# themayflyman/yet-another-raytracer

Hardware: AMD Instinct MI355X
Metric: Msamples/sec (WxHxspp/sec), cornell-box 800x800x256spp depth 50 (higher is better)
Workload: dtype f64; 1 GPU; cornell-box 800x800x256spp depth 50 (BASELINE configs[1]); width=800, height=800, spp=256, max_depth=50, parallelism=pixel-blocks x1, launch=one process, one GPU, streams=2, prep_frames=0, full=False, seed=1497453140, build_id=b5b5abf84520346f09e41dc92cfc8f159110369d6109f06c5935a081cd03fc2a

## Files before the change

yet-another-raytracer_amd/csrc/kernels.hip:

```cpp
#include <hip/hip_runtime.h>
#include <math.h>
#include <type_traits>

#include "kernels.h"

namespace yart_dev {

__constant__ double c_cie[471][3] = {
#include "cie_xyz.inc"
};
constexpr double kMinLambda = 360.0, kMaxLambda = 720.0, kBinWidth = 10.0;
constexpr double kCieYIntegral = 106.856895;
constexpr double kMaxLum = 20.0;
constexpr double kPi = 3.141592653589793;
constexpr double kEps = 2.220446049250313e-16;
constexpr double kF64Max = 1.7976931348623157e308;

struct V3 { double x, y, z; };
__device__ __forceinline__ V3 mk(double x, double y, double z) { return V3{x, y, z}; }
__device__ __forceinline__ V3 add(V3 a, V3 b) { return mk(a.x + b.x, a.y + b.y, a.z + b.z); }
__device__ __forceinline__ V3 sub(V3 a, V3 b) { return mk(a.x - b.x, a.y - b.y, a.z - b.z); }
__device__ __forceinline__ V3 muls(V3 a, double s) { return mk(a.x * s, a.y * s, a.z * s); }
__device__ __forceinline__ V3 smul(double s, V3 a) { return mk(s * a.x, s * a.y, s * a.z); }
__device__ __forceinline__ V3 neg(V3 a) { return mk(-a.x, -a.y, -a.z); }
// ... 1532 lines not shown
      cx(0, 1); cx(2, 3); cx(0, 2); cx(1, 3); cx(1, 2);
      if (key[0] < INFINITY) {
        if (key[3] < INFINITY) stk[(cursor++) * 64] = hc[3];
        if (key[2] < INFINITY) stk[(cursor++) * 64] = hc[2];
        if (key[1] < INFINITY) stk[(cursor++) * 64] = hc[1];
        hnd = hc[0];
      } else {
        if (cursor == 0) break;
        cursor--;
        hnd = stk[cursor * 64];
      }
    }
  }
  id.obj = who >> 3; id.sub = who & 7u;
  id.t = closest;
  return found;
}

template <bool HAS_MESH, bool BVH, bool STATS, bool EXT, int SLOTS = kCoopSlots, bool OVF = false, bool PARK = false>
__device__ __forceinline__ bool world_hit(const DevScene& S, bool want, const Ray& r, double tmin, double tmax, Hit& rec,
                                          int32_t& which, uint32_t* stk, uint8_t* coop, Stats& st, const QueryCtx& q,
                                          uint32_t* ovf = nullptr, bool resume = false, bool* parked = nullptr) {
  HitId id;
  if constexpr (BVH) {
    if (!world_closest_bvh<STATS>(S, r, tmin, tmax, id, stk, st)) return false;
  } else {
    if (!world_closest<HAS_MESH, STATS, EXT, SLOTS, OVF, PARK>(S, want, r, tmin, tmax, id, stk, coop, st, q, ovf, resume, parked) ||
        !want || (PARK && *parked))
      return false;
  }
  hit_record<HAS_MESH, EXT>(S, r, id, rec);
  which = (int32_t)id.obj;
  return true;
}


struct Onb { V3 v, w; };
template <class M>
__device__ __forceinline__ Onb onb_from_w(V3 n, M& m) {
  Onb b;
  b.w = m.unit(n);
  const V3 a = fabs(b.w.x) > 0.9 ? mk(0.0, 1.0, 0.0) : mk(1.0, 0.0, 0.0);
  b.v = m.unit(cross(b.w, a));
  return b;
}
__device__ __forceinline__ V3 local(const Onb& b, V3 a) {
  const V3 u = cross(b.w, b.v);
  return add(add(smul(a.x, u), smul(a.y, b.v)), smul(a.z, b.w));
}
template <class M>
__device__ __forceinline__ V3 random_cosine_direction(Rng& g, M& m) {
  const double r1 = gen_f64(g), r2 = gen_f64(g);
  const double z = m.sqrt(1.0 - r2);
  double s, c;
  sincos_det(2.0 * kPi * r1, s, c);
  const double sr2 = m.sqrt(r2);
  return mk(c * sr2, s * sr2, z);
}
template <bool CDIV, class M>
__device__ __forceinline__ double over_pi(double x, M& m) {
  if (!CDIV || !YART_CONST_DIV) return x / kPi;
  double d = kPi, r = kRcpPi;
  asm volatile("" : "+s"(d), "+s"(r));
  return m.quo(x, PosDen{d, r});
}
template <bool CDIV, class M>
__device__ __forceinline__ double cosine_value(const Onb& b, V3 ud, M& m) {
  const double cosine = dot(ud, b.w);
  return cosine <= 0.0 ? 0.0 : over_pi<CDIV>(cosine, m);
}

template <bool LEN, class M>
__device__ __forceinline__ double light_pdf_at(const DevObject& o, V3 origin, V3 dir, double ldir, bool hit, double t, M& m) {
  if (!hit) return 0.0;
  if (o.kind == YART_PRIM_XZ_RECT) {
    Hit h;
    rect_rec(1, Ray{origin, dir, 0.0, 0.0}, t, h);
    const double area = (o.p[1] - o.p[0]) * (o.p[3] - o.p[2]);
    const double distance_squared = h.t * h.t * len2(dir);
    const double cosine = fabs(dot(dir, h.n)) / (LEN ? m.len(dir) : ldir);
    return distance_squared / (cosine * area);
  }
  const double radius = o.p[3];
  const double cos_theta_max = m.sqrt(1.0 - radius * radius / len2(sub(ld3(o.p), origin)));
  const double solid_angle = 2.0 * kPi * (1.0 - cos_theta_max);
  return 1.0 / solid_angle;
}
template <bool STATS, bool LEN, class M>
__device__ __forceinline__ double light_pdf(const DevObject& o, V3 origin, V3 dir, double ldir, double wl, Stats& st, M& m) {
  if (o.n_xf != 0) return 0.0;
  Ray r{origin, dir, 0.0, wl};
  double t = 0.0;
  bool hit;
  if (o.kind == YART_PRIM_XZ_RECT) {
    if (STATS) st.v[ST_LIGHT]++;
    hit = rect_t<1, 0, 2>(o.p, r, 0.001, INFINITY, t);
  } else if (o.kind == YART_PRIM_SPHERE) {
    if (STATS) st.v[ST_LIGHT]++;
    hit = sphere_t(o.p, r, 0.001, INFINITY, t, m);
  } else {
    return 0.0;
  }
  return light_pdf_at<LEN>(o, origin, dir, ldir, hit, t, m);
}
template <class M>
__device__ __forceinline__ V3 light_random(const DevObject& o, V3 origin, Rng& g, M& m) {
  if (o.n_xf == 0 && o.kind == YART_PRIM_XZ_RECT) {
    const double x = gen_range(g, o.p[0], o.p[1]);
    const double z = gen_range(g, o.p[2], o.p[3]);
    return sub(mk(x, o.p[4], z), origin);
  }
  if (o.n_xf == 0 && o.kind == YART_PRIM_SPHERE) {
    const V3 direction = sub(ld3(o.p), origin);
    const double d2 = len2(direction);
    const Onb uvw = onb_from_w(direction, m);
    const double r1 = gen_f64(g), r2 = gen_f64(g);
    const double radius = o.p[3];
    const double z = 1.0 + r2 * (m.sqrt(1.0 - radius * radius / d2) - 1.0);
    double s, c;
    sincos_det(2.0 * kPi * r1, s, c);
    const double sz = m.sqrt(1.0 - z * z);
    const V3 rs = mk(c * sz, s * sz, z);
    return local(uvw, rs);
  }
  return mk(1.0, 0.0, 0.0);
}

__device__ __forceinline__ int32_t sat_i32(double f) {
  if (f != f) return 0;
  if (f >= 2147483647.0) return INT32_MAX;
  if (f <= -2147483648.0) return INT32_MIN;
  return (int32_t)f;
}
__device__ __noinline__ double perlin_noise(const yart_perlin* P, uint32_t type, V3 p) {
  if (type == YART_NOISE_SQUARE) {
    const int32_t i = sat_i32(4.0 * p.x) & 255, j = sat_i32(4.0 * p.y) & 255, k = sat_i32(4.0 * p.z) & 255;
    return P->ranfloat[P->perm_x[i] ^ P->perm_y[j] ^ P->perm_z[k]];
  }
  double u = p.x - floor(p.x), v = p.y - floor(p.y), w = p.z - floor(p.z);
  const uint32_t i = (uint32_t)sat_i32(floor(p.x)), j = (uint32_t)sat_i32(floor(p.y)), k = (uint32_t)sat_i32(floor(p.z));
  double accum = 0.0;
  if (type == YART_NOISE_TRILINEAR) {
    u = u * u * (3.0 - 2.0 * u);
    v = v * v * (3.0 - 2.0 * v);
    w = w * w * (3.0 - 2.0 * w);
    for (uint32_t di = 0; di < 2; ++di)
      for (uint32_t dj = 0; dj < 2; ++dj)
        for (uint32_t dk = 0; dk < 2; ++dk) {
          const double c = P->ranfloat[P->perm_x[(i + di) & 255u] ^ P->perm_y[(j + dj) & 255u] ^ P->perm_z[(k + dk) & 255u]];
          accum += ((double)di * u + (double)(1u - di) * (1.0 - u)) * ((double)dj * v + (double)(1u - dj) * (1.0 - v)) *
                   ((double)dk * w + (double)(1u - dk) * (1.0 - w)) * c;
        }
    return accum;
  }
  const double uu = u * u * (3.0 - 2.0 * u), vv = v * v * (3.0 - 2.0 * v), ww = w * w * (3.0 - 2.0 * w);
  for (uint32_t di = 0; di < 2; ++di)
    for (uint32_t dj = 0; dj < 2; ++dj)
      for (uint32_t dk = 0; dk < 2; ++dk) {
        const double* c = P->ranvec[P->perm_x[(i + di) & 255u] ^ P->perm_y[(j + dj) & 255u] ^ P->perm_z[(k + dk) & 255u]];
        const V3 weight_v = mk(u - (double)di, v - (double)dj, w - (double)dk);
        accum += ((double)di * uu + (1.0 - (double)di) * (1.0 - uu)) * ((double)dj * vv + (1.0 - (double)dj) * (1.0 - vv)) *
                 ((double)dk * ww + (1.0 - (double)dk) * (1.0 - ww)) * dot(weight_v, ld3(c));
      }
  return accum;
}
__device__ __forceinline__ double perlin_turb(const yart_perlin* P, uint32_t type, V3 p, int depth) {
  double accum = 0.0, weight = 1.0;
  V3 temp_p = p;
  for (int d = 0; d < depth; ++d) {
    accum += weight * perlin_noise(P, type, temp_p);
    weight *= 0.5;
    temp_p = muls(temp_p, 2.0);
  }
  return fabs(accum);
}

__constant__ double c_smits[7][36] = {
#include "smits.inc"
};
__device__ __forceinline__ double rgb_reflect(double red, double green, double blue, int i) {
  enum { W, Cy, Ma, Ye, Re, Gr, Bl };
  double s = 0.0;
  if (red <= green && red <= blue) {
    s = red * c_smits[W][i] + s;
    if (green <= blue) { s = (green - red) * c_smits[Cy][i] + s; s = (blue - green) * c_smits[Bl][i] + s; }
    else { s = (blue - red) * c_smits[Cy][i] + s; s = (green - blue) * c_smits[Gr][i] + s; }
  } else if (green <= red && green <= blue) {
    s = green * c_smits[W][i] + s;
    if (red <= blue) { s = (red - green) * c_smits[Ma][i] + s; s = (blue - red) * c_smits[Bl][i] + s; }
    else { s = (blue - green) * c_smits[Ma][i] + s; s = (red - blue) * c_smits[Re][i] + s; }
  } else {
    s = blue * c_smits[W][i] + s;
    if (red <= green) { s = (red - blue) * c_smits[Ye][i] + s; s = (green - red) * c_smits[Gr][i] + s; }
    else { s = (green - blue) * c_smits[Ye][i] + s; s = (red - green) * c_smits[Re][i] + s; }
  }
  return s;
}
__device__ __forceinline__ double clampd(double x, double lo, double hi) { return x < lo ? lo : (x > hi ? hi : x); }
__device__ __forceinline__ uint32_t sat_u32(double f) {
  if (!(f > 0.0)) return 0u;
  if (f >= 4294967295.0) return 0xFFFFFFFFu;
  return (uint32_t)f;
}

template <bool EXT>
__device__ __forceinline__ double texture_value(const DevScene& S, uint32_t ti, int bin, V3 p, double hu = 0.0,
                                                double hv = 0.0) {
  const DevTexture& t = S.textures[ti];
  if (EXT && t.kind == YART_TEX_IMAGE) {
    if (!t.pixels || t.width == 0 || t.height == 0) return 1.0;
    const double uu = clampd(hu, 0.0, 1.0), vv = 1.0 - clampd(hv, 0.0, 1.0);
    uint32_t i = sat_u32(uu * (double)t.width), j = sat_u32(vv * (double)t.height);
    if (i >= t.width) i = t.width - 1;
    if (j >= t.height) j = t.height - 1;
    const double color_scale = 1.0 / 255.0;
    const uint8_t* px = t.pixels + (size_t)j * t.width * 3 + (size_t)i * 3;
    return rgb_reflect(color_scale * (double)px[0], color_scale * (double)px[1], color_scale * (double)px[2], bin);
  }
  if (EXT && t.kind == YART_TEX_NOISE) {
    const double white = t.spec[bin];
    if (t.noise_type == YART_NOISE_NET) return white * perlin_turb(t.perlin, t.noise_type, muls(p, t.scale), 7);
    if (t.noise_type == YART_NOISE_MARBLE)
      return white * 0.5 * (1.0 + sin_det(t.scale * p.z + 10.0 * perlin_turb(t.perlin, t.noise_type, p, 7)));
    return white * 0.5 * (1.0 + perlin_noise(t.perlin, t.noise_type, muls(p, t.scale)));
  }
  if (t.kind == YART_TEX_CHECKER) {
    const double sines = sin_det(10.0 * p.x) * sin_det(10.0 * p.y) * sin_det(10.0 * p.z);
    return sines < 0.0 ? t.spec[bin] : t.spec_even[bin];
  }
  return t.spec[bin];
}
__device__ __forceinline__ V3 reflect(V3 v, V3 n) { return sub(v, smul(2.0 * dot(v, n), n)); }

constexpr size_t kKernargCam = (sizeof(DevScene) + alignof(RenderArgs) - 1) / alignof(RenderArgs) * alignof(RenderArgs) +
                               offsetof(RenderArgs, cam);
typedef const __attribute__((address_space(4))) yart_camera* kcam_ptr;
__device__ __forceinline__ kcam_ptr kernarg_camera() {
  const __attribute__((address_space(4))) char* p =
      (const __attribute__((address_space(4))) char*)__builtin_amdgcn_kernarg_segment_ptr();
  asm volatile("" : "+s"(p));
  return (kcam_ptr)(p + kKernargCam);
}
__device__ __forceinline__ V3 ld3(const __attribute__((address_space(4))) double* p) { return mk(p[0], p[1], p[2]); }
#ifndef YART_KA_OPAQUE
#define YART_KA_OPAQUE 1
#endif
typedef const __attribute__((address_space(4))) RenderArgs* kargs_ptr;
template <bool OPAQUE>
__device__ __forceinline__ kargs_ptr kernarg_args() {
  const __attribute__((address_space(4))) char* p =
      (const __attribute__((address_space(4))) char*)__builtin_amdgcn_kernarg_segment_ptr();
  if (OPAQUE) asm volatile("" : "+s"(p));
  return (kargs_ptr)(p + (kKernargCam - offsetof(RenderArgs, cam)));
}

template <class Cam>
__device__ __forceinline__ Ray camera_ray(const Cam& c, double s, double t, double wl, Rng& g,
                                          bool draw_time) {
  const V3 org = ld3(c.origin);
  const V3 d0 = sub(add(add(ld3(c.lower_left_corner), smul(s, ld3(c.horizontal))), smul(t, ld3(c.vertical))), org);
  Ray r;
  r.wl = wl;
  if (c.lens_radius == 0.0 && !draw_time && org.x != 0.0 && org.y != 0.0 && org.z != 0.0 && d0.x != 0.0 &&
      d0.y != 0.0 && d0.z != 0.0) {
    r.o = org;
    r.d = d0;
    r.time = c.time0;
    return r;
  }
  V3 p;
  for (int guard = 0; guard < 1024; ++guard) {
    const double x = gen_range(g, -1.0, 1.0);
    const double y = gen_range(g, -1.0, 1.0);
    p = mk(x, y, 0.0);
    if (!(len2(p) >= 1.0)) break;
  }
  const V3 rd = smul(c.lens_radius, p);
  const V3 offset = add(muls(ld3(c.u), rd.x), muls(ld3(c.v), rd.y));
  r.o = add(org, offset);
  r.d = sub(d0, offset);
  r.time = draw_time ? gen_range(g, c.time0, c.time1) : c.time0;
  return r;
}

__device__ __forceinline__ bool covered(uint32_t x, uint32_t w) {
  asm volatile("" : "+s"(w));
  const uint32_t cw = w / 8;
#pragma unroll
  for (uint32_t col = 0; col < 8; ++col) {
    const uint32_t x0 = (uint32_t)(((uint64_t)w * col) / 8);
    if (x >= x0 && x < x0 + cw) return true;
  }
  return false;
}

__device__ __forceinline__ uint32_t xcd_remap(uint32_t b, uint32_t n) {
  const uint32_t q = n / 8, r = n % 8, xcd = b % 8, k = b / 8;
  return (xcd < r ? xcd * (q + 1) : r * (q + 1) + (xcd - r) * q) + k;
}

constexpr int kWavesPerEu = 4;
constexpr int kMeshWavesPerEu = 4;

template <bool EXT, bool STATS, bool SHARE, class MP>
__device__ __forceinline__ void scatter_at(const DevScene& S, MP& mp, Rng& g, const V3& hp, const V3& hn, uint32_t hmat,
                                           double hu, double hv, int wbin, const Ray& ray, double T, uint32_t depth,
                                           Stats& st, double& T_, V3& o_, V3& d_, uint32_t& depth_, double& R_,
                                           bool& term_) {
  T_ = T; o_ = hp; d_ = ray.d; depth_ = depth; R_ = 0.0; term_ = false;
  const DevMaterial& m = S.materials[hmat];
  const uint32_t kind = m.kind;
  if (kind == YART_MAT_LAMBERTIAN) {
    auto att = [&]() { return texture_value<EXT>(S, m.texture, wbin, hp, hu, hv); };
    const Onb uvw = onb_from_w(hn, mp);
    V3 dir, udir;
    double ldir;
    double pdf_val;
    if (S.n_lights == 0) {
      (void)gen_range(g, 0.0, 1.0);
      dir = local(uvw, random_cosine_direction(g, mp));
      udir = mp.unit_len(dir, ldir);
      pdf_val = 0.5 * cosine_value<SHARE && !EXT>(uvw, udir, mp) + 0.5 * cosine_value<SHARE && !EXT>(uvw, udir, mp);
    } else {
      if (gen_range(g, 0.0, 1.0) < 0.5) {
        if (S.n_lights <= 2) {
          dir = light_random(uniform_at(S.lights, 0u), hp, g, mp);
        } else {
          const uint32_t k = (uint32_t)gen_index(g, S.n_lights - 1);
          dir = light_random(S.lights[k], hp, g, mp);
        }
      } else {
        dir = local(uvw, random_cosine_direction(g, mp));
      }
      const double weight = 1.0 / (double)S.n_lights;
      double sum = -0.0;
      if (SHARE) udir = mp.unit_len(dir, ldir);
      else ldir = 0.0;
      for (uint32_t i = 0; i < S.n_lights; ++i)
        sum = sum + weight * light_pdf<STATS, !SHARE>(uniform_at(S.lights, i), hp, dir, ldir, ray.wl, st, mp);
      if (!SHARE) udir = mp.unit(dir);
      pdf_val = 0.5 * sum + 0.5 * cosine_value<SHARE && !EXT>(uvw, udir, mp);
    }
    if (!isfinite(pdf_val) || pdf_val <= 0.0) {
      R_ = T * 0.0;
      term_ = true;
    } else {
      const double cosine = dot(hn, SHARE ? udir : mp.unit(dir));
      const double spdf = cosine < 0.0 ? 0.0 : over_pi<SHARE && !EXT>(cosine, mp);
      T_ = ((T * att()) * spdf) / pdf_val;
      o_ = hp;
      d_ = dir;
      depth_ = depth - 1;
    }
  } else if (EXT && kind == YART_MAT_ISOTROPIC) {
    const double att = texture_value<EXT>(S, m.texture, wbin, hp, hu, hv);
    V3 p;
    for (int guard = 0; guard < 1024; ++guard) {
      const double px = gen_range(g, -1.0, 1.0), py = gen_range(g, -1.0, 1.0), pz = gen_range(g, -1.0, 1.0);
      p = mk(px, py, pz);
      if (!(len2(p) >= 1.0)) break;
    }
    T_ = T * att;
    o_ = hp;
    d_ = p;
    depth_ = depth - 1;
  } else if (kind == YART_MAT_METAL) {
    const V3 reflected = reflect(mp.unit(ray.d), hn);
    V3 p;
    for (int guard = 0; guard < 1024; ++guard) {
      const double px = gen_range(g, -1.0, 1.0), py = gen_range(g, -1.0, 1.0), pz = gen_range(g, -1.0, 1.0);
      p = mk(px, py, pz);
      if (!(len2(p) >= 1.0)) break;
    }
    const double att = texture_value<EXT>(S, m.texture, wbin, hp, hu, hv);
    T_ = T * att;
    o_ = hp;
    d_ = add(reflected, smul(m.fuzz, p));
    depth_ = depth - 1;
  } else {
    const double wl2 = ray.wl * ray.wl;
    const double n2 = 1.0 + m.b[0] * wl2 / (wl2 - m.c[0]) + m.b[1] * wl2 / (wl2 - m.c[1]) + m.b[2] * wl2 / (wl2 - m.c[2]);
    const double n = mp.sqrt(n2);
    const PosDen ld = mp.den(mp.len(ray.d));
    V3 outward;
    double ni_over_nt, cosine;
    if (dot(ray.d, hn) > 0.0) {
      outward = neg(hn); ni_over_nt = n; cosine = mp.quo(n * dot(ray.d, hn), ld);
    } else {
      outward = hn; ni_over_nt = 1.0 / n; cosine = mp.quo(-dot(ray.d, hn), ld);
    }
    const V3 uv = mk(mp.quo(ray.d.x, ld), mp.quo(ray.d.y, ld), mp.quo(ray.d.z, ld));
    const double dt = dot(uv, outward);
    const double disc = 1.0 - ni_over_nt * ni_over_nt * (1.0 - dt * dt);
    V3 out;
    if (disc > 0.0) {
      const V3 refracted = sub(muls(sub(uv, muls(outward, dt)), ni_over_nt), muls(outward, mp.sqrt(disc)));
      double r0 = (1.0 - n) / (1.0 + n);
      r0 = r0 * r0;
      const double sch = r0 + (1.0 - r0) * powi5(1.0 - cosine);
      out = gen_f64(g) < sch ? reflect(ray.d, hn) : refracted;
    } else {
      out = reflect(ray.d, hn);
    }
    T_ = T * 1.0;
    o_ = hp;
    d_ = out;
    depth_ = depth - 1;
  }
}

template <bool HAS_MESH, bool BVH, bool STATS, bool DYN, bool EXT, bool DEEP = false>
__global__ __launch_bounds__(256, HAS_MESH ? kMeshWavesPerEu : kWavesPerEu) void k_render(DevScene S, RenderArgs A_) {
#if YART_KA_OPAQUE
#define A (*kernarg_args<!BVH>())
#else
#define A A_
#endif
  __shared__ uint32_t s_stack[HAS_MESH ? 4 * kWaveLdsWords : BVH ? 4 * kStackSlots * 64 : 1];
  constexpr bool JOBL = DYN && !HAS_MESH, JOBL3 = DYN && HAS_MESH;
  constexpr bool PARK = HAS_MESH && DYN && !EXT && !DEEP;
  __shared__ uint32_t s_job[JOBL ? 4 * 6 * 64 : JOBL3 ? 4 * 3 * 64 : 1];
  const uint32_t lane = threadIdx.x & 63u, wave = __builtin_amdgcn_readfirstlane(threadIdx.x >> 6);
  uint32_t work = DYN ? 0u : xcd_remap(blockIdx.x, gridDim.x) * 4 + wave;
  if (!DYN && work >= A.n_blocks * A.n_chunks) return;
  uint32_t local_blk = work % A.n_blocks, chunk_id = work / A.n_blocks;
  uint32_t b = A.shard_index + local_blk * A.shard_count;
  uint32_t bx0 = (b % A.blocks_x) * 8, by0 = (b / A.blocks_x) * 8;
  uint32_t slot = lane;
  uint32_t x = bx0 + (slot & 7u), y = by0 + (slot >> 3);
  const uint32_t W = A.width, H = A.height;
  const bool active = x < W && y < H && covered(x, W) && covered(y, H);
  uint32_t* const jl = &s_job[JOBL ? wave * 6 * 64 + lane : JOBL3 ? wave * 3 * 64 + lane : 0];
  constexpr bool JL = JOBL || JOBL3;
  uint32_t* stk = &s_stack[HAS_MESH ? (wave * kWaveLdsWords + lane) : BVH ? (wave * kStackSlots * 64 + lane) : 0];
  uint8_t* coop = reinterpret_cast<uint8_t*>(&s_stack[HAS_MESH ? wave * kWaveLdsWords : 0]);
  uint32_t* const ovf = (DEEP || PARK) ? A.stack_ovf + (size_t)(blockIdx.x * 4u + wave) * kOvfWords : nullptr;
  if (PARK) {
    if (lane < 16u) reinterpret_cast<uint32_t*>(coop + coop_bytes<kCoopSlots>() + 64)[lane] = 0u;
    __builtin_amdgcn_fence(__ATOMIC_SEQ_CST, "wavefront");
  }
  Stats st;
  if (STATS) for (int i = 0; i < kNumStats; ++i) st.v[i] = 0;

  uint32_t pixel = y * W + x;
  double acc0 = 0.0, acc1 = 0.0, acc2 = 0.0;
  const uint32_t s_end = A.s_begin + A.s_count;
  uint32_t s_lo = A.s_begin + chunk_id * A.chunk;
  const uint32_t s_stop = s_lo + A.chunk < s_end ? s_lo + A.chunk : s_end;
  uint32_t smp = s_lo;
  uint32_t lane_blk = local_blk;
  uint32_t n_jobs = 0, next_job = 0;
  uint64_t cov = 0;
  bool drained = false;
  bool need = true;
  bool parked = false;
  bool alive = DYN ? true : (active && smp < s_stop);
  Rng g;
  Ray ray;
  double T = 1.0;
  uint32_t depth = 0;
  bool fresh = !DYN && alive;
  V3 hp = mk(0.0, 0.0, 0.0), hn = hp;
  uint32_t hmat = 0;
  double hu = 0.0, hv = 0.0;
  int wbin = 0;
  g.k0 = (uint32_t)A.seed; g.k1 = (uint32_t)(A.seed >> 32);

  for (;;) {
    if (DYN) {
      uint64_t m = drained ? 0ull : __ballot(need);
      while (m) {
        if (next_job >= n_jobs) {
          const uint32_t first = (uint32_t)__builtin_ctzll(__ballot(true));
          uint32_t v = 0;
          if (lane == first) {
            if (HAS_MESH) {
              v = 0xFFFFFFFFu;
              const uint32_t x0 = blockIdx.x & 7u;
              for (uint32_t k = 0; k < 8u; ++k) {
                const uint32_t x = (x0 + k) & 7u;
                const uint32_t lo = (uint32_t)(((uint64_t)A.n_units * x) >> 3);
                const uint32_t hi = (uint32_t)(((uint64_t)A.n_units * (x + 1u)) >> 3);
                if (hi <= lo) continue;
                const uint32_t t = atomicAdd(A.queue + 1 + x, 1u);
                if (t < hi - lo) { v = lo + t; break; }
              }
              if (A.progress) {
                const uint32_t c = v < A.n_units ? atomicAdd(A.queue, 1u) + 1u : A.n_units;
                __hip_atomic_store(A.progress, A.progress_base + (c < A.n_units ? c : A.n_units), __ATOMIC_RELAXED,
                                   __HIP_MEMORY_SCOPE_SYSTEM);
              }
            } else {
              v = atomicAdd(A.queue, 1u);
              if (A.progress)
                __hip_atomic_store(A.progress, A.progress_base + (v < A.n_units ? v + 1u : A.n_units), __ATOMIC_RELAXED,
                                   __HIP_MEMORY_SCOPE_SYSTEM);
            }
          }
          const uint32_t u = (uint32_t)__builtin_amdgcn_readlane((int)v, (int)first);
          if (u >= A.n_units) { drained = true; break; }
          local_blk = u / A.n_chunks; chunk_id = u % A.n_chunks;
          b = A.shard_index + local_blk * A.shard_count;
          bx0 = (b % A.blocks_x) * 8; by0 = (b / A.blocks_x) * 8;
          s_lo = A.s_begin + chunk_id * A.chunk;
          const uint32_t stop = s_lo + A.chunk < s_end ? s_lo + A.chunk : s_end;
          n_jobs = (stop > s_lo ? stop - s_lo : 0) * 64;
          next_job = 0;
          {
            const uint32_t cx = bx0 + (lane & 7u), cy = by0 + (lane >> 3);
            cov = __ballot(cx < W && cy < H && covered(cx, W) && covered(cy, H));
          }
          continue;
        }
        const uint32_t rank = __builtin_amdgcn_mbcnt_hi((uint32_t)(m >> 32), __builtin_amdgcn_mbcnt_lo((uint32_t)m, 0u));
        const uint32_t avail = n_jobs - next_job;
        if (need && rank < avail) {
          const uint32_t job = next_job + rank;
          slot = job & 63u;
          smp = s_lo + (job >> 6);
          x = bx0 + (slot & 7u);
          y = by0 + (slot >> 3);
          pixel = y * W + x;
          lane_blk = local_blk;
          if (JOBL) { jl[0] = pixel; jl[64] = smp; jl[128] = lane_blk; jl[192] = slot; jl[256] = x; jl[320] = y; }
          if (JOBL3) { jl[0] = pixel; jl[64] = smp; jl[128] = lane_blk; }
          if ((cov >> slot) & 1ull) { fresh = true; need = false; }
        }
        const uint32_t given = (uint32_t)__popcll(m);
        next_job += given < avail ? given : avail;
        m = __ballot(need);
      }
    }
    const bool run = DYN ? !need : alive;
    if (__ballot(run) == 0) break;
    bool term = false, want = PARK && parked;
    if (STATS) {
      const uint64_t cam = __ballot(run && fresh), sca = __ballot(run && !fresh);
      if (lane == 0) {
        st.v[ST_ITERS]++;
        st.v[ST_CAMERA_LANES] += (uint32_t)__popcll(cam);
        st.v[ST_SCATTER_LANES] += (uint32_t)__popcll(sca);
        st.v[ST_CAMERA_ITERS] += cam ? 1u : 0u;
        st.v[ST_SCATTER_ITERS] += sca ? 1u : 0u;
      }
    }
    if (run && !(PARK && parked)) {
      rng_phase<!HAS_MESH && !BVH>(g, JL ? jl[0] : pixel, JL ? jl[64] : smp, fresh ? 0u : A.max_depth - depth + 1u);
      if (fresh) {
        uint32_t jx = x, jy = y;
        if (JOBL) { jx = jl[256]; jy = jl[320]; }
        if (JOBL3) { const uint32_t p = jl[0]; jy = p / W; jx = p - jy * W; }
        uint32_t wm1 = W - 1, hm1 = H - 1;
        asm volatile("" : "+s"(wm1), "+s"(hm1));
        const double tx = (double)jx + gen_f64(g);
        const double u = tx / (double)wm1;
        const double ty = (double)jy + gen_f64(g);
        const double v = 1.0 - ty / (double)hm1;
        const double wl = gen_range(g, kMinLambda, kMaxLambda);
        ray = camera_ray(*kernarg_camera(), u, v, wl, g, EXT && S.has_time);
        wbin = spectrum_bin<!HAS_MESH && !EXT>(wl);
        T = 1.0;
        depth = A.max_depth;
        fresh = false;
      } else {
        auto scatter = [&](auto& mp, double& T_, V3& o_, V3& d_, uint32_t& depth_, double& R_, bool& term_) {
          scatter_at<EXT, STATS, !HAS_MESH>(S, mp, g, hp, hn, hmat, hu, hv, wbin, ray, T, depth, st, T_, o_, d_, depth_, R_, term_);
        };
        double nT, nR;
        V3 no, nd;
        uint32_t ndepth;
        bool nterm;
        typename MathPolicy<HAS_MESH, BVH, EXT>::type fm;
        scatter(fm, nT, no, nd, ndepth, nR, nterm);
        if (flagged(fm)) {
          rng_phase<!HAS_MESH && !BVH>(g, JL ? jl[0] : pixel, JL ? jl[64] : smp, A.max_depth - depth + 1u);
          Ieee im;
          scatter(im, nT, no, nd, ndepth, nR, nterm);
        }
        T = nterm ? nR : nT; ray.o = no; ray.d = nd; depth = ndepth; term = nterm;
      }
      if (!term) {
        if (depth == 0) {
          T = T * 1.0;
          term = true;
        } else {
          want = true;
        }
      }
    }
    {
      Hit h;
      int32_t which;
      bool hit = false;
      bool scat = false;
      const QueryCtx q{g.k0, g.k1, JL ? jl[64] : smp, JL ? jl[0] : pixel, A.max_depth - depth + 1u};
      if (HAS_MESH) {
        bool now = false;
        hit = world_hit<HAS_MESH, BVH, STATS, EXT, kCoopSlots, DEEP, PARK>(S, want, ray, 0.001, INFINITY, h, which, stk, coop, st, q,
                                                                          ovf, parked, &now);
        if (PARK) {
          parked = now;
          want = want && !now;
        }
      } else if (want) {
        hit = world_hit<HAS_MESH, BVH, STATS, EXT>(S, true, ray, 0.001, INFINITY, h, which, stk, coop, st, q);
      }
      if (want && !term) {
        if (STATS) st.v[ST_SEGMENTS]++;
        if (!hit) {
          T = T * S.background[wbin];
          term = true;
        } else {
          const DevMaterial& m = S.materials[h.mat];
          const uint32_t kind = m.kind;
          if (kind == YART_MAT_LAMBERTIAN || kind == YART_MAT_METAL || kind == YART_MAT_DIELECTRIC ||
              (EXT && kind == YART_MAT_ISOTROPIC)) {
            scat = true;
          } else {
            double emitted = 0.0;
            if (kind == YART_MAT_DIFFUSE_LIGHT && h.ff) emitted = texture_value<EXT>(S, m.texture, wbin, h.p, h.u, h.v);
            T = T * emitted;
            term = true;
          }
        }
      }
      hp = scat ? h.p : mk(0.0, 0.0, 0.0);
      hn = scat ? h.n : mk(0.0, 0.0, 0.0);
      hmat = scat ? h.mat : 0u;
      if (EXT) { hu = scat ? h.u : 0.0; hv = scat ? h.v : 0.0; }
    }
    if (run && term) {
      const double R = T;
      double cx, cy, cz;
      cie_xyz(ray.wl, cx, cy, cz);
      double sx = cx * R, sy = cy * R, sz = cz * R;
      if (!isfinite(sx) || !isfinite(sy) || !isfinite(sz)) {
        sx = sy = sz = 0.0;
      } else if (!(sy <= 0.0 || sy <= kMaxLum)) {
        const double k = kMaxLum / sy;
        sx = sx * k; sy = sy * k; sz = sz * k;
      }
      if (STATS) st.v[ST_SAMPLES]++;
      if (DYN) {
        const uint32_t jb = JL ? jl[128] : lane_blk, js = JL ? jl[64] : smp;
        uint32_t jsl = JOBL ? jl[192] : slot;
        if (JOBL3) {
          const uint32_t p = jl[0], py = p / W, px = p - py * W;
          jsl = (py & 7u) * 8u + (px & 7u);
        }
        double* q = A.scratch + 3 * (((size_t)jb * A.s_count + (js - A.s_begin)) * 64 + jsl);
        q[0] = sx; q[1] = sy; q[2] = sz;
        need = true;
      } else {
        acc0 = acc0 + sx; acc1 = acc1 + sy; acc2 = acc2 + sz;
        smp++;
        if (smp < s_stop) fresh = true;
        else alive = false;
      }
    }
  }
  if (!DYN && active) {
    double* o = A.out + 3 * (A.packed ? (size_t)local_blk * 64 + lane : (size_t)pixel);
    o[0] = acc0; o[1] = acc1; o[2] = acc2;
  }
  if (!DYN && A.progress && lane == 0) {
    const uint32_t done = atomicAdd(A.progress_count, 1u) + 1u;
    __hip_atomic_store(A.progress, A.progress_base + done, __ATOMIC_RELAXED, __HIP_MEMORY_SCOPE_SYSTEM);
  }
  if (STATS) {
    for (int i = 0; i < kNumStats; ++i)
      if (st.v[i]) atomicAdd(&A.stats[i], st.v[i]);
  }
}

#undef A

__device__ __forceinline__ void wf_job(const RenderArgs& A, uint32_t job, uint32_t& pixel, uint32_t& smp, uint32_t& x,
                                       uint32_t& y) {
  const uint32_t slot = job & 63u, rest = job >> 6;
  const uint32_t blk = rest / A.s_count, s = rest - blk * A.s_count;
  const uint32_t b = A.shard_index + blk * A.shard_count;
  x = (b % A.blocks_x) * 8u + (slot & 7u);
  y = (b / A.blocks_x) * 8u + (slot >> 3);
  pixel = y * A.width + x;
  smp = A.s_begin + s;
}
__device__ __forceinline__ void wf_store_sample(const RenderArgs& A, uint32_t job, double wl, double R) {
  double cx, cy, cz;
  cie_xyz(wl, cx, cy, cz);
  double sx = cx * R, sy = cy * R, sz = cz * R;
  if (!isfinite(sx) || !isfinite(sy) || !isfinite(sz)) {
    sx = sy = sz = 0.0;
  } else if (!(sy <= 0.0 || sy <= kMaxLum)) {
    const double k = kMaxLum / sy;
    sx = sx * k; sy = sy * k; sz = sz * k;
  }
  double* q = A.scratch + 3 * (size_t)job;
  q[0] = sx; q[1] = sy; q[2] = sz;
}

__global__ __launch_bounds__(256) void k_wf_shade(DevScene S, RenderArgs A, WfArgs F) {
  __shared__ uint32_t s_need[4], s_take[3];
  const uint32_t i = blockIdx.x * 256u + threadIdx.x;
  const uint32_t lane = threadIdx.x & 63u, wave = __builtin_amdgcn_readfirstlane(threadIdx.x >> 6);
  const uint32_t P = F.pool;
  const uint32_t W = A.width, H = A.height;
  const WfSlots& Q = F.q;
  Stats st;
  Rng g;
  g.k0 = (uint32_t)A.seed; g.k1 = (uint32_t)(A.seed >> 32);
  Ray ray;
  ray.time = 0.0;
  ray.wl = 0.0;
  ray.o = mk(0.0, 0.0, 0.0); ray.d = ray.o;
  double T = 0.0;
  uint32_t job = Q.job[i], depth = 0;
  bool has = false;
  if (job != kWfNoJob) {
    depth = Q.depth[i]; T = Q.T[i]; ray.wl = Q.wl[i];
    ray.o = mk(Q.o[i], Q.o[P + i], Q.o[2 * (size_t)P + i]);
    ray.d = mk(Q.d[i], Q.d[P + i], Q.d[2 * (size_t)P + i]);
    const int wbin = spectrum_bin<false>(ray.wl);
    const uint32_t obj = Q.hobj[i];
    double R = 0.0;
    bool term = false;
    if (obj == kWfMiss) {
      R = T * S.background[wbin];
      term = true;
    } else {
      HitId id;
      id.t = Q.ht[i]; id.u = Q.hu[i]; id.v = Q.hv[i]; id.obj = obj; id.sub = Q.hsub[i];
      Hit h;
      hit_record<true, false>(S, ray, id, h);
      const DevMaterial& m = S.materials[h.mat];
      const uint32_t kind = m.kind;
      if (kind == YART_MAT_LAMBERTIAN || kind == YART_MAT_METAL || kind == YART_MAT_DIELECTRIC) {
        uint32_t pixel, smp, x, y;
        wf_job(A, job, pixel, smp, x, y);
        rng_phase<false>(g, pixel, smp, A.max_depth - depth + 1u);
        double nT, nR;
        V3 no, nd;
        uint32_t ndepth;
        bool nterm;
        Ieee im;
        scatter_at<false, false, false>(S, im, g, h.p, h.n, h.mat, 0.0, 0.0, wbin, ray, T, depth, st, nT, no, nd, ndepth, nR, nterm);
        if (nterm) {
          R = nR;
          term = true;
        } else if (ndepth == 0) {
          R = nT * 1.0;
          term = true;
        } else {
          T = nT; ray.o = no; ray.d = nd; depth = ndepth;
          has = true;
        }
      } else {
        double emitted = 0.0;
        if (kind == YART_MAT_DIFFUSE_LIGHT && h.ff) emitted = texture_value<false>(S, m.texture, wbin, h.p);
        R = T * emitted;
        term = true;
      }
    }
    if (term) wf_store_sample(A, job, ray.wl, R);
  }
  bool need = !has;
  uint32_t next = 0, end = 0;
  if (threadIdx.x == 0) { next = Q.range[2 * blockIdx.x]; end = Q.range[2 * blockIdx.x + 1]; }
  for (;;) {
    if (!__syncthreads_or(need)) break;
    const uint64_t m = __ballot(need);
    if (lane == 0) s_need[wave] = (uint32_t)__popcll(m);
    __syncthreads();
    const uint32_t total = s_need[0] + s_need[1] + s_need[2] + s_need[3];
    uint32_t before = 0;
    for (uint32_t w = 0; w < wave; ++w) before += s_need[w];
    if (threadIdx.x == 0) {
      uint32_t base = kWfNoJob;
      if (end - next < total && *(volatile uint32_t*)F.jobs < F.total_jobs) {
        base = atomicAdd(F.jobs, kWfChunk);
        if (base >= F.total_jobs) base = kWfNoJob;
      }
      s_take[0] = next; s_take[1] = base;
      const uint32_t rem = end - next;
      if (base != kWfNoJob) {
        next = base + (total - rem);
        end = base + kWfChunk < F.total_jobs ? base + kWfChunk : F.total_jobs;
        if (next > end) next = end;
      } else {
        next += rem < total ? rem : total;
      }
      s_take[2] = rem;
    }
    __syncthreads();
    const uint32_t from = s_take[0], base = s_take[1], rem = s_take[2];
    const bool dry = base == kWfNoJob && rem < total;
    if (need) {
      const uint32_t r = before + __builtin_amdgcn_mbcnt_hi((uint32_t)(m >> 32), __builtin_amdgcn_mbcnt_lo((uint32_t)m, 0u));
      uint32_t jb = kWfNoJob;
      if (r < rem) jb = from + r;
      else if (base != kWfNoJob && base + (r - rem) < F.total_jobs) jb = base + (r - rem);
      if (jb == kWfNoJob) {
        need = false;
        job = kWfNoJob;
      } else {
        uint32_t pixel, smp, x, y;
        wf_job(A, jb, pixel, smp, x, y);
        if (x < W && y < H && covered(x, W) && covered(y, H)) {
          job = jb;
          rng_phase<false>(g, pixel, smp, 0u);
          const double tx = (double)x + gen_f64(g);
          const double u = tx / (double)(W - 1);
          const double ty = (double)y + gen_f64(g);
          const double v = 1.0 - ty / (double)(H - 1);
          const double wl = gen_range(g, kMinLambda, kMaxLambda);
          ray = camera_ray(*kernarg_camera(), u, v, wl, g, false);
          ray.time = 0.0;
          T = 1.0;
          depth = A.max_depth;
          if (depth == 0) {
            wf_store_sample(A, job, ray.wl, T * 1.0);
          } else {
            has = true;
            need = false;
          }
        }
      }
    }
    if (dry) {
      need = false;
      if (!has) job = kWfNoJob;
    }
    __syncthreads();
  }
  if (threadIdx.x == 0) { Q.range[2 * blockIdx.x] = next; Q.range[2 * blockIdx.x + 1] = end; }
  Q.job[i] = has ? job : kWfNoJob;
  if (has) {
    Q.o[i] = ray.o.x; Q.o[P + i] = ray.o.y; Q.o[2 * (size_t)P + i] = ray.o.z;
    Q.d[i] = ray.d.x; Q.d[P + i] = ray.d.y; Q.d[2 * (size_t)P + i] = ray.d.z;
    Q.T[i] = T; Q.wl[i] = ray.wl; Q.depth[i] = depth;
  }
  if (__syncthreads_or(has) && threadIdx.x == 0) *F.alive = 1u;
}

constexpr int kWfTraceWaves = 4;
template <int SLOTS>
__global__ __launch_bounds__(64, SLOTS == kCoopSlots ? kWfTraceWaves : 3) void k_wf_trace(DevScene S, RenderArgs A,
                                                                                            WfArgs F) {
  constexpr int kWords = wave_lds_words<SLOTS>();
  __shared__ uint32_t s_stack[kWords];
  if (blockIdx.x == 0 && threadIdx.x == 0) {
    const uint32_t v = *F.alive;
    *F.alive_next = 0u;
    __hip_atomic_store(F.status, v, __ATOMIC_RELAXED, __HIP_MEMORY_SCOPE_SYSTEM);
  }
  const uint32_t lane = threadIdx.x, P = F.pool;
  uint32_t* stk = &s_stack[lane];
  uint8_t* coop = reinterpret_cast<uint8_t*>(&s_stack[0]);
  for (uint32_t bt = blockIdx.x; bt < P / 64u; bt += P) {
    const uint32_t i = bt * 64u + lane;
    const bool want = F.q.job[i] != kWfNoJob;
    if (__ballot(want) == 0) continue;
    Ray r;
    r.o = mk(F.q.o[i], F.q.o[P + i], F.q.o[2 * (size_t)P + i]);
    r.d = mk(F.q.d[i], F.q.d[P + i], F.q.d[2 * (size_t)P + i]);
    r.time = 0.0; r.wl = 0.0;
    HitId id;
    Stats st;
    const QueryCtx q{0u, 0u, 0u, 0u, 0u};
    const bool hit = world_closest<true, false, false, SLOTS>(S, want, r, 0.001, INFINITY, id, stk, coop, st, q);
// ... 239 lines not shown
```

Baseline: 5963 Msamples/s.

## Batch camera rays per wave and park in-flight scatter paths in LDS

```diff
diff --git a/yet-another-raytracer_amd/csrc/kernels.hip b/yet-another-raytracer_amd/csrc/kernels.hip
--- a/yet-another-raytracer_amd/csrc/kernels.hip
+++ b/yet-another-raytracer_amd/csrc/kernels.hip
@@ -1858,11 +1858,11 @@
 constexpr int kWavesPerEu = 4;
 constexpr int kMeshWavesPerEu = 4;
 
-template <bool EXT, bool STATS, bool SHARE, class MP>
+template <bool EXT, bool STATS, bool SHARE, bool OPQ = false, class MP>
 __device__ __forceinline__ void scatter_at(const DevScene& S, MP& mp, Rng& g, const V3& hp, const V3& hn, uint32_t hmat,
                                            double hu, double hv, int wbin, const Ray& ray, double T, uint32_t depth,
                                            Stats& st, double& T_, V3& o_, V3& d_, uint32_t& depth_, double& R_,
-                                           bool& term_) {
+                                           bool& term_, double lweight = 0.0) {
   T_ = T; o_ = hp; d_ = ray.d; depth_ = depth; R_ = 0.0; term_ = false;
   const DevMaterial& m = S.materials[hmat];
   const uint32_t kind = m.kind;
@@ -1882,13 +1882,18 @@
         if (S.n_lights <= 2) {
           dir = light_random(uniform_at(S.lights, 0u), hp, g, mp);
         } else {
-          const uint32_t k = (uint32_t)gen_index(g, S.n_lights - 1);
+          uint32_t nl1 = S.n_lights - 1;
+          if (OPQ) {
+            nl1 = __builtin_amdgcn_readfirstlane(nl1);
+            asm volatile("" : "+s"(nl1));
+          }
+          const uint32_t k = (uint32_t)gen_index(g, nl1);
           dir = light_random(S.lights[k], hp, g, mp);
         }
       } else {
         dir = local(uvw, random_cosine_direction(g, mp));
       }
-      const double weight = 1.0 / (double)S.n_lights;
+      const double weight = OPQ ? lweight : 1.0 / (double)S.n_lights;
       double sum = -0.0;
       if (SHARE) udir = mp.unit_len(dir, ldir);
       else ldir = 0.0;
@@ -1975,7 +1980,15 @@
   __shared__ uint32_t s_stack[HAS_MESH ? 4 * kWaveLdsWords : BVH ? 4 * kStackSlots * 64 : 1];
   constexpr bool JOBL = DYN && !HAS_MESH, JOBL3 = DYN && HAS_MESH;
   constexpr bool PARK = HAS_MESH && DYN && !EXT && !DEEP;
-  __shared__ uint32_t s_job[JOBL ? 4 * 6 * 64 : JOBL3 ? 4 * 3 * 64 : 1];
+  constexpr bool PRIM = DYN && !HAS_MESH && !BVH && !EXT;
+  constexpr int kRecF64 = 11, kRecU32 = 6, kJobWords = PRIM ? 4 : 6;
+  __shared__ uint32_t s_job[JOBL ? 4 * kJobWords * 64 : JOBL3 ? 4 * 3 * 64 : 1];
+  __shared__ double s_recd[PRIM ? 4 * kRecF64 * 64 : 1];
+  __shared__ uint32_t s_recu[PRIM ? 4 * kRecU32 * 64 : 1];
+  static_assert(!PRIM || kWavesPerEu * (sizeof(s_job) + sizeof(s_recd) + sizeof(s_recu)) <= 160u * 1024u,
+                "k_render (PRIM): the parked-path buffers and job words of kWavesPerEu workgroups exceed the CU's LDS");
+  static_assert(!HAS_MESH || kMeshWavesPerEu * (sizeof(s_stack) + sizeof(s_job)) <= 160u * 1024u,
+                "k_render (mesh): the walk state and job words of kMeshWavesPerEu workgroups exceed the CU's LDS");
   const uint32_t lane = threadIdx.x & 63u, wave = __builtin_amdgcn_readfirstlane(threadIdx.x >> 6);
   uint32_t work = DYN ? 0u : xcd_remap(blockIdx.x, gridDim.x) * 4 + wave;
   if (!DYN && work >= A.n_blocks * A.n_chunks) return;
@@ -1986,7 +1999,11 @@
   uint32_t x = bx0 + (slot & 7u), y = by0 + (slot >> 3);
   const uint32_t W = A.width, H = A.height;
   const bool active = x < W && y < H && covered(x, W) && covered(y, H);
-  uint32_t* const jl = &s_job[JOBL ? wave * 6 * 64 + lane : JOBL3 ? wave * 3 * 64 + lane : 0];
+  uint32_t* const jl = &s_job[JOBL ? wave * kJobWords * 64 + lane : JOBL3 ? wave * 3 * 64 + lane : 0];
+  double* const recd = &s_recd[PRIM ? wave * kRecF64 * 64 : 0];
+  uint32_t* const recu = &s_recu[PRIM ? wave * kRecU32 * 64 : 0];
+  uint32_t rec_n = 0;
+  bool batch = false;
   constexpr bool JL = JOBL || JOBL3;
   uint32_t* stk = &s_stack[HAS_MESH ? (wave * kWaveLdsWords + lane) : BVH ? (wave * kStackSlots * 64 + lane) : 0];
   uint8_t* coop = reinterpret_cast<uint8_t*>(&s_stack[HAS_MESH ? wave * kWaveLdsWords : 0]);
@@ -2022,8 +2039,85 @@
   int wbin = 0;
   g.k0 = (uint32_t)A.seed; g.k1 = (uint32_t)(A.seed >> 32);
 
+  double lweight = 0.0;
+  if (PRIM) {
+    const double w = 1.0 / (double)S.n_lights;
+    const uint32_t lo = __builtin_amdgcn_readfirstlane(lo_word(w)), hi = __builtin_amdgcn_readfirstlane((uint32_t)hi_word(w));
+    lweight = __longlong_as_double((long long)(((uint64_t)hi << 32) | lo));
+  }
+
   for (;;) {
-    if (DYN) {
+    if constexpr (PRIM) {
+      uint64_t m = (drained && rec_n == 0u) ? 0ull : __ballot(need);
+      batch = false;
+      while (m) {
+        if (rec_n == 0u) {
+          if (drained) break;
+          if (next_job >= n_jobs) {
+            const uint32_t first = (uint32_t)__builtin_ctzll(__ballot(true));
+            uint32_t v = 0;
+            if (lane == first) {
+              v = atomicAdd(A.queue, 1u);
+              if (A.progress)
+                __hip_atomic_store(A.progress, A.progress_base + (v < A.n_units ? v + 1u : A.n_units), __ATOMIC_RELAXED,
+                                   __HIP_MEMORY_SCOPE_SYSTEM);
+            }
+            const uint32_t u = (uint32_t)__builtin_amdgcn_readlane((int)v, (int)first);
+            if (u >= A.n_units) { drained = true; break; }
+            local_blk = u / A.n_chunks; chunk_id = u % A.n_chunks;
+            b = A.shard_index + local_blk * A.shard_count;
+            bx0 = (b % A.blocks_x) * 8; by0 = (b / A.blocks_x) * 8;
+            s_lo = A.s_begin + chunk_id * A.chunk;
+            const uint32_t stop = s_lo + A.chunk < s_end ? s_lo + A.chunk : s_end;
+            n_jobs = (stop > s_lo ? stop - s_lo : 0) * 64;
+            next_job = 0;
+            const uint32_t cx = bx0 + (lane & 7u), cy = by0 + (lane >> 3);
+            cov = __ballot(cx < W && cy < H && covered(cx, W) && covered(cy, H));
+            if (cov == 0ull) n_jobs = 0;
+            continue;
+          }
+          {
+            const uint64_t pm = __ballot(!need);
+            if (!need) {
+              const uint32_t e = __builtin_amdgcn_mbcnt_hi((uint32_t)(pm >> 32), __builtin_amdgcn_mbcnt_lo((uint32_t)pm, 0u));
+              recd[e] = hp.x; recd[64 + e] = hp.y; recd[128 + e] = hp.z;
+              recd[192 + e] = hn.x; recd[256 + e] = hn.y; recd[320 + e] = hn.z;
+              recd[384 + e] = ray.d.x; recd[448 + e] = ray.d.y; recd[512 + e] = ray.d.z;
+              recd[576 + e] = ray.wl; recd[640 + e] = T;
+              recu[e] = hmat; recu[64 + e] = ((uint32_t)wbin << 6) | jl[192];
+              recu[128 + e] = jl[0]; recu[192 + e] = jl[64]; recu[256 + e] = jl[128]; recu[320 + e] = depth;
+            }
+            rec_n = (uint32_t)__popcll(pm);
+          }
+          jl[0] = (by0 + (lane >> 3)) * W + bx0 + (lane & 7u);
+          jl[64] = s_lo + (next_job >> 6); jl[128] = local_blk; jl[192] = lane;
+          next_job += 64u;
+          batch = true;
+          need = !((cov >> lane) & 1ull);
+          hp = mk(0.0, 0.0, 0.0); hn = hp; hmat = 0u;
+          __builtin_amdgcn_fence(__ATOMIC_SEQ_CST, "wavefront");
+          break;
+        }
+        const uint32_t rank = __builtin_amdgcn_mbcnt_hi((uint32_t)(m >> 32), __builtin_amdgcn_mbcnt_lo((uint32_t)m, 0u));
+        if (need && rank < rec_n) {
+          const uint32_t e = rec_n - 1u - rank;
+          hp = mk(recd[e], recd[64 + e], recd[128 + e]);
+          hn = mk(recd[192 + e], recd[256 + e], recd[320 + e]);
+          ray.d = mk(recd[384 + e], recd[448 + e], recd[512 + e]);
+          ray.wl = recd[576 + e]; T = recd[640 + e];
+          hmat = recu[e];
+          const uint32_t bs = recu[64 + e];
+          wbin = (int)(bs >> 6);
+          jl[0] = recu[128 + e]; jl[64] = recu[192 + e]; jl[128] = recu[256 + e]; jl[192] = bs & 63u;
+          depth = recu[320 + e];
+          need = false;
+        }
+        const uint32_t given = (uint32_t)__popcll(m);
+        rec_n -= given < rec_n ? given : rec_n;
+        m = __ballot(need);
+      }
+    }
+    if (DYN && !PRIM) {
       uint64_t m = drained ? 0ull : __ballot(need);
       while (m) {
         if (next_job >= n_jobs) {
@@ -2088,10 +2182,11 @@
       }
     }
     const bool run = DYN ? !need : alive;
+    const bool start = PRIM ? batch : fresh;
     if (__ballot(run) == 0) break;
     bool term = false, want = PARK && parked;
     if (STATS) {
-      const uint64_t cam = __ballot(run && fresh), sca = __ballot(run && !fresh);
+      const uint64_t cam = __ballot(run && start), sca = __ballot(run && !start);
       if (lane == 0) {
         st.v[ST_ITERS]++;
         st.v[ST_CAMERA_LANES] += (uint32_t)__popcll(cam);
@@ -2101,10 +2196,11 @@
       }
     }
     if (run && !(PARK && parked)) {
-      rng_phase<!HAS_MESH && !BVH>(g, JL ? jl[0] : pixel, JL ? jl[64] : smp, fresh ? 0u : A.max_depth - depth + 1u);
-      if (fresh) {
+      rng_phase<!HAS_MESH && !BVH>(g, JL ? jl[0] : pixel, JL ? jl[64] : smp, start ? 0u : A.max_depth - depth + 1u);
+      if (start) {
         uint32_t jx = x, jy = y;
-        if (JOBL) { jx = jl[256]; jy = jl[320]; }
+        if (JOBL && !PRIM) { jx = jl[256]; jy = jl[320]; }
+        if (PRIM) { jx = bx0 + (lane & 7u); jy = by0 + (lane >> 3); }
         if (JOBL3) { const uint32_t p = jl[0]; jy = p / W; jx = p - jy * W; }
         uint32_t wm1 = W - 1, hm1 = H - 1;
         asm volatile("" : "+s"(wm1), "+s"(hm1));
@@ -2120,7 +2216,7 @@
         fresh = false;
       } else {
         auto scatter = [&](auto& mp, double& T_, V3& o_, V3& d_, uint32_t& depth_, double& R_, bool& term_) {
-          scatter_at<EXT, STATS, !HAS_MESH>(S, mp, g, hp, hn, hmat, hu, hv, wbin, ray, T, depth, st, T_, o_, d_, depth_, R_, term_);
+          scatter_at<EXT, STATS, !HAS_MESH, PRIM>(S, mp, g, hp, hn, hmat, hu, hv, wbin, ray, T, depth, st, T_, o_, d_, depth_, R_, term_, lweight);
         };
         double nT, nR;
         V3 no, nd;
```

Measured after the change: 7324 Msamples/s, median of 6. +22.8%, better.
